# AlexanderFengler/hddm

Measured on AMD Instinct MI355X. Metric: trial-likelihood evals/sec (full DDM, sv/sz/st) at 1/2/4/8 GPUs, higher is better.
Workload: dtype f64; 1 GPU; C3: full DDM 1M trials on 1 GPU; trials_per_gpu=1000000, global_trials=1000000, parallelism=trial-shard x1

## Files before the change

hddm_amd/_lib.py:

```python
import ctypes
import os
import threading

import numpy as np

_PKG = os.path.dirname(os.path.abspath(__file__))
LIB_PATH = os.environ.get("WFPT_AMD_LIB", os.path.join(_PKG, "lib", "libwfpt_amd.so"))

if not os.path.exists(LIB_PATH):
    raise ImportError(
        f"hddm_amd: HIP library not found at {LIB_PATH}; build it with "
        "`python -m hddm_amd.build` (hipcc --offload-arch=gfx950)")

os.environ.setdefault("HIP_FORCE_DEV_KERNARG", "1")

_lib = ctypes.CDLL(LIB_PATH)

WFPT_OK = 0
WFPT_MAX_DEPTH = 24
WFPT_DS_INPUT_ORDER = 1
PATH_LEAN, PATH_ENGINE, PATH_SMALL, PATH_REDO = 1, 2, 4, 8
PATH_FOLD, PATH_DIRECT, PATH_FIXED, PATH_SPLIT = 16, 32, 64, 128
PATH_SMALL_SPLIT, PATH_NODE_SPLIT, PATH_NODE_RARE = 256, 512, 1024
LINK_IDENTITY, LINK_EXP, LINK_INVLOGIT = 0, 1, 2
# ... 71 lines not shown
    "wfpt_wiener_like_host": (_I, [_VP, _PD, _I64, _PP, _PK, _PD]),
    "wfpt_pdf_array": (_I, [_VP, _PD, _I64, _PP, _PK, _I, _PD]),
    "wfpt_full_pdf": (_I, [_VP, _D, _PP, _PK, _PD]),
    "wfpt_wiener_like_multi": (_I, [_VP, _PD, _I64] + _MULTI),
    "wfpt_wiener_like_multi_ex": (_I, [_VP, _PD, _I64] + _MULTI + [_PD]),
    "wfpt_dmat_cdf_array": (_I, [_VP, _PD, _I64, _PP, _D, _PD]),
    "wfpt_dmat_cdf_rows": (_I, [_VP, _PP, _PD, _PD, _PD, _I64, _I32, _D, _PD, _PD, _PD]),
    "wfpt_comm_unique_id": (_I, [_CP]),
    "wfpt_comm_init": (_I, [_VP, _I, _I, _CP]),
    "wfpt_comm_exchange_id": (_I, [_I, _I, _CP, _I, _I, _CP]),
    "wfpt_comm_init_tcp": (_I, [_VP, _I, _I, _CP, _I, _I]),
    "wfpt_comm_init_all": (_I, [_PVP, _I]),
    "wfpt_wiener_like_allreduce": (_I, _LIKE),
    "wfpt_wiener_like_allreduce_group": (_I, [_PVP, _PVP, _I, _PP, _PK, _PD]),
    "wfpt_wiener_like_nodes_allreduce": (_I, [_VP, _VP, _PP, _I32, _PK, _PD]),
    "wfpt_result_poison": (_I, [_PD]),
    "wfpt_decode_result": (_I, [_PD, _PD]),
    "wfpt_profile_enable": (_I, [_VP, _I]),
    "wfpt_profile_read": (_I, [_VP, _PD, _PI64, _PI64, _I]),
    "wfpt_profile_stages": (_I, [_VP, _PD, _I]),
    "wfpt_profile_lists": (_I, [_VP, _PI64, _I]),
    "wfpt_debug_waves": (_I, [_VP, _PU64, _I64]),
    "wfpt_debug_partials": (_I, [_VP, _PD, _PI32, _I64]),
    "wfpt_last_path": (_I, [_VP, _PI]),
    "wfpt_rl_dataset_create": (_I, [_VP, _PD, _PI64, _PD, _PI64, _I64, _PI32, _I32, _PVP]),
    "wfpt_rl_dataset_destroy": (None, [_VP]),
    "wfpt_wiener_like_rlddm": (_I, [_VP, _VP, _D, _D, _D, _PP, _PK, _PD]),
    "wfpt_wiener_like_rlddm_ex": (_I, [_VP, _VP, _D, _D, _D, _PP, _PK, _PD, _PD, _PD]),
    "wfpt_wiener_like_rl": (_I, [_VP, _VP] + [_D] * 7 + [_PD]),
    "wfpt_wiener_like_rl_ex": (_I, [_VP, _VP] + [_D] * 7 + [_PD, _PD, _PD]),
    "wfpt_wiener_like_multi_rlddm": (_I, _RL_HOST + _MULTI),
    "wfpt_wiener_like_multi_rlddm_ex": (_I, _RL_HOST + _MULTI + [_PD, _PD]),
    "wfpt_wiener_like_rlddm_nodes": (_I, [_VP, _VP, _PD, _PP, _PK, _PD]),
    "wfpt_wiener_like_rlddm_nodes_ex": (_I, [_VP, _VP, _PD, _PP, _PK, _PD, _PD, _PD]),
    "wfpt_wiener_like_rlddm_nodes_multi": (_I, [_VP, _VP, _PD, _PP, _I32, _PK, _PD]),
    "wfpt_wiener_like_rlddm_nodes_multi_ex": (_I, [_VP, _VP, _PD, _PP, _I32, _PK, _PD, _PD, _PD]),
    "wfpt_reg_dataset_create": (_I, [_VP, _PD, _I64, _PD, _I32, _PI32, _I32, _PVP]),
    "wfpt_reg_dataset_destroy": (None, [_VP]),
    "wfpt_wiener_like_reg": (_I, _REG),
    "wfpt_wiener_like_reg_ex": (_I, _REG + [_PD, _PD]),
    "wfpt_wiener_like_reg_groups": (_I, _REG),
    "wfpt_wiener_like_reg_groups_ex": (_I, _REG + [_PD, _PD]),
    "wfpt_rl_reg_dataset_create": (_I, [_VP, _PD, _PI64, _PD, _PI64, _I64, _PD, _I32, _PI32, _I32,
                                        _PVP]),
    "wfpt_rl_reg_dataset_destroy": (None, [_VP]),
    "wfpt_wiener_like_rl_reg_groups": (_I, _RL_REG),
# ... 130 lines not shown
        a = (_I64 * 16)()
        if wfpt_profile_lists is None:
            return {}
        check(wfpt_profile_lists(self.handle, a, 1 if reset else 0))
        v = list(a)
        return {"segments": v[0], "lean_table": v[0], "node_deferred": v[3], "lean_generic": v[3],
                "tasks1": v[1], "tasks2": v[2], "records": v[4], "exact": v[5],
                "walk": v[6], "zwalks": v[7], "zwalks0": v[8], "zwalks1": v[9],
                "zwalks2": v[10], "phase_kcycles": v[11:16]}

    def debug_waves(self, n):
        out = np.zeros((n, 8), dtype=np.uint64)
        check(wfpt_debug_waves(self.handle, out.ctypes.data_as(_PU64), n))
        return out

    def synchronize(self):
        check(wfpt_synchronize(self.handle))

    def last_path(self):
        v = _I()
        check(wfpt_last_path(self.handle, ctypes.byref(v)))
        return v.value

    def partials(self, n):
        part = np.empty(n, dtype=np.float64)
        zero = np.empty(n, dtype=np.int32)
        check(wfpt_debug_partials(self.handle, dptr(part), zero.ctypes.data_as(_PI32), n))
        return part, zero


_ctx_lock = threading.Lock()
_contexts = {}


def default_device():
    env = os.environ.get("WFPT_DEVICE")
    if env is not None:
        return int(env)
    return 0


def context(device=None):
    dev = default_device() if device is None else int(device)
    with _ctx_lock:
        c = _contexts.get(dev)
        if c is None:
# ... 26 lines not shown
```

hddm_amd/csrc/capi_core.cpp:

```cpp
#include <cstdio>

#include "capi_internal.hpp"
#include "rl_internal.h"

using namespace wfpt::capi;

constexpr int64_t kSplitCap = 16384;
constexpr int64_t kHeavyFewDiv = 16;

namespace wfpt {
namespace capi {

thread_local std::string g_last_error;

int fail(int code, const std::string& msg) {
  g_last_error = msg;
  return code;
}

bool roctx_on() {
  static const bool on = [] {
    const char* e = std::getenv("WFPT_ROCTX");
    return !(e && std::strcmp(e, "0") == 0);
  }();
  return on;
}

void ds_register(wfpt_ctx* c, DsBase* d) {
  d->ctx = c;
  c->dsets.push_back(d);
}
// ... 107 lines not shown
}

static const wfpt::DecisionTab* decision_tab_of(wfpt_ctx* c, double err) {
  uint64_t key;
  std::memcpy(&key, &err, sizeof key);
  if (!c->dtab_valid || c->dtab_err != key) {
    if (err > 1e-30 && err < 1e30) wfpt::decision_tab(err, c->dtab);
    else wfpt::decision_tab_clear(c->dtab);
    c->dtab_err = key;
    c->dtab_valid = true;
  }
  return &c->dtab;
}

int run_sum(wfpt_ctx* c, const double* dx, int64_t n, const wfpt::Params& P,
            const wfpt::Knobs& K, double* out, int part, const wfpt_ds* d,
            double* mirror) {
  const int64_t nb = wfpt::partials_for(n, P, K);
  HIP_TRY(c->part.reserve(std::max<int64_t>(nb, 1)));
  HIP_TRY(c->zero.reserve(std::max<int64_t>(nb, 1)));
  wfpt::Work W;
  if (int rc = reserve_work(c, n, &W)) return rc;
  const bool adaptive = wfpt::has_deferred_pass(P, K);
  if (part & wfpt::kPassFast) c->path = 0;
  if (c->count && (part & wfpt::kPassFast))
    HIP_TRY(hipMemsetAsync(c->evals.p, 0, sizeof(unsigned long long), c->stream));
  const bool prof = c->profile && (part & wfpt::kPassFast);
  if (prof) HIP_TRY(hipEventRecord(c->ev0, c->stream));
  const bool eng = d && d->hcount.p && engine_family(P, K) &&
                   !(part & (wfpt::kPassLean | wfpt::kPassRedo));
  const bool level0_only = adaptive && (engine_family(P, K)
                                            ? part == (wfpt::kPassFast | wfpt::kPassLean)
                                            : part == wfpt::kPassFast);
  const bool direct = adaptive && !engine_family(P, K);
  if (c->small && level0_only && !prof && !c->count && !mirror) {
    const int sk = wfpt::launch_small(dx, n, P, K, c->part.p, c->zero.p, c->status.p, W, out,
                                      c->seq + 1, c->tree_any.p, c->stream, c->trial);
    if (sk != wfpt::kSmallNone) {
      ++c->seq;
      HIP_TRY(hipGetLastError());
      c->path |= WFPT_PATH_SMALL | (direct ? WFPT_PATH_DIRECT : WFPT_PATH_LEAN) |
                 (sk == wfpt::kSmallSplit ? WFPT_PATH_SMALL_SPLIT : 0);
      return WFPT_OK;
    }
  }
  const wfpt::Split S = eng ? split_of(d) : wfpt::Split{};
  wfpt::launch_trials(c->trial ? 3 : 0, adaptive ? part : wfpt::kPassAll, dx, n, P, K, c->part.p,
                      c->zero.p, c->count ? c->evals.p : nullptr, c->status.p, 0, W, c->stream,
                      prof ? c->ev1 : nullptr, &S, c->trial,
                      ((part & wfpt::kPassLean) &&
                       wfpt::select_mode(P.sz, P.st, K.use_adaptive) == wfpt::kAdaptTZ)
                          ? decision_tab_of(c, K.err)
                          : nullptr);
  if (!adaptive) {
    c->path |= WFPT_PATH_FIXED;
  } else {
    if (part & wfpt::kPassFast)
      c->path |= direct ? WFPT_PATH_DIRECT
                        : (part & wfpt::kPassLean)
                              ? WFPT_PATH_LEAN
                              : (WFPT_PATH_ENGINE | (S.n + S.n2 > 0 ? WFPT_PATH_SPLIT : 0));
    if (!direct && (part & wfpt::kPassRedo)) c->path |= WFPT_PATH_REDO;
    if (part & wfpt::kPassDeferred) c->path |= WFPT_PATH_FOLD;
  }
  HIP_TRY(hipGetLastError());
  wfpt::launch_finalize(c->part.p, c->zero.p, nb, adaptive ? 1 : 0,
                        c->status.p, out, ++c->seq, c->stream, eng ? S.next_n : nullptr,
                        eng ? d->hcount.p + d->parity : nullptr, c->tree_any.p, mirror, c->fin.p,
                        c->fin_ticket.p);
  HIP_TRY(hipGetLastError());
  return WFPT_OK;
}

int finish_profile(wfpt_ctx* c) {
  if (c->profile) {
    float ms = 0.f;
// ... 194 lines not shown

int wfpt_open(int device, wfpt_ctx** out) {
  if (!out) return fail(WFPT_ERR_ARG, "null pointer");
  int nd = 0;
  HIP_TRY(hipGetDeviceCount(&nd));
  if (device < 0 || device >= nd)
    return fail(WFPT_ERR_ARG, "device " + std::to_string(device) + " not present (" +
                                  std::to_string(nd) + " visible)");
  DeviceGuard g(device);
  HIP_TRY(hipSetDevice(device));
  auto* c = new wfpt_ctx();
  c->device = device;
  if (const char* sm = std::getenv("WFPT_SYNC")) c->spin = std::strcmp(sm, "stream") != 0;
  if (const char* nm = std::getenv("WFPT_NODES")) c->nodes_generic = std::strcmp(nm, "generic") == 0;
  if (const char* ns = std::getenv("WFPT_NODE_SPLIT")) c->node_split = std::strcmp(ns, "0") != 0;
  if (const char* nq = std::getenv("WFPT_NODE_SPEC")) c->node_spec = std::strcmp(nq, "0") != 0;
  if (const char* ht = std::getenv("WFPT_HOST_TIMING")) c->host_timing = std::strcmp(ht, "0") != 0;
  if (const char* nt = std::getenv("WFPT_NODE_TABLE_DEV"))
    c->node_table_dev = std::strcmp(nt, "0") != 0;
  if (const char* fm = std::getenv("WFPT_FAST_ONLY")) c->fast_only = std::strcmp(fm, "0") != 0;
  if (const char* lm = std::getenv("WFPT_LEAN")) c->lean = std::strcmp(lm, "0") != 0;
  if (const char* sm = std::getenv("WFPT_SMALL")) c->small = std::strcmp(sm, "0") != 0;
  if (const char* lt = std::getenv("WFPT_LEAN_TREE")) c->lean_tree_max = std::atof(lt);
  hipError_t e = hipStreamCreateWithFlags(&c->stream, hipStreamNonBlocking);
  if (e == hipSuccess) e = hipEventCreate(&c->ev0);
  if (e == hipSuccess) e = hipEventCreate(&c->ev1);
  auto words = [&](auto& b, size_t n) {
    if (e == hipSuccess) e = b.reserve(n);
    if (e == hipSuccess) e = hipMemset(b.p, 0, n * sizeof(*b.p));
  };
  words(c->evals, 1), words(c->status, 1), words(c->n_defer, 4), words(c->ncnt, 4);
  words(c->tree_any, 1), words(c->fin, 3 * 64), words(c->fin_ticket, 1), words(c->ar, 8);
  words(c->prof, 16), words(c->phase, 8 * wfpt::kPhaseWaves);
  if (e == hipSuccess) e = c->host_status.reserve(1);
  if (e == hipSuccess) e = c->mres.reserve(8);
  if (e == hipSuccess) std::memset(c->mres.h, 0, 8 * sizeof(double));
  if (e != hipSuccess) {
    wfpt_close(c);
    return fail(WFPT_ERR_HIP, std::string("wfpt_open: ") + hipGetErrorString(e));
  }
  *out = c;
  return WFPT_OK;
}

void wfpt_close(wfpt_ctx* c) {
  if (!c) return;
// ... 57 lines not shown
    for (int64_t i = 0; i < n; ++i) ord[i] = i;
    if (!keep_order) stable_order(ord, rt, false);
    std::vector<int64_t> pos(cnt.begin(), cnt.end() - 1);
    for (int64_t q : ord) idx[pos[node_id[q]]++] = q;
  } else if (!keep_order) {
    stable_order(idx, rt, true);
  }
  std::vector<double> hx(n);
  std::vector<int32_t> hn(node_id ? n : 0);
  for (int64_t i = 0; i < n; ++i) {
    hx[i] = rt[idx[i]];
    if (node_id) hn[i] = node_id[idx[i]];
  }
  auto* d = new wfpt_ds();
  d->n = n;
  d->input_order = (flags & WFPT_DS_INPUT_ORDER) != 0;
  d->n_nodes = node_id ? n_nodes : 0;
  hipError_t e = upload_vec(d->x, hx);
  d->identity = !((!keep_order || node_id) && n > 0);
  if (e == hipSuccess && !d->identity) e = upload_vec(d->perm, idx);
  if (e == hipSuccess && node_id) e = upload_vec(d->node, hn);
  if (e == hipSuccess && node_id) e = upload_vec(d->off, off);
  d->nw = (n + 63) / 64;
  d->split_cap = (int)std::min<int64_t>(std::max<int64_t>(d->nw, 1), kSplitCap);
  const size_t cap = d->split_cap;
  auto zeroed = [&](auto& b, size_t count) {
    if (e == hipSuccess) e = b.reserve(count);
    if (e == hipSuccess) e = hipMemset(b.p, 0, count * sizeof(*b.p));
  };
  for (int k = 0; k < 2; ++k) {
    zeroed(d->hpred[k], std::max<int64_t>(d->nw, 1));
    if (e == hipSuccess) e = d->hlist[k].reserve(cap);
  }
  zeroed(d->hcount, 4);
  if (e == hipSuccess) e = d->hlp.reserve(cap * 64);
  if (e == hipSuccess) e = d->hmeta.reserve(cap * 64);
  zeroed(d->hdone, cap);
  zeroed(d->hzn, cap);
  if (e != hipSuccess) {
    delete d;
    return fail(WFPT_ERR_HIP, std::string("wfpt_dataset_create: ") + hipGetErrorString(e));
  }
  ds_register(c, d);
  *out = d;
  return WFPT_OK;
}
// ... 790 lines not shown
  HIP_TRY(hipMemcpy(ph.data(), c->phase.p, ph.size() * sizeof(ph[0]), hipMemcpyDeviceToHost));
  for (int k = 0; k < 5; ++k) {
    unsigned long long t = 0;
    for (int w = 0; w < wfpt::kPhaseWaves; ++w) t += ph[w * 8 + 2 + k];
    counts[11 + k] = (int64_t)(t / 1000);
  }
  if (reset) {
    HIP_TRY(hipMemset(c->prof.p, 0, sizeof(h)));
    HIP_TRY(hipMemset(c->phase.p, 0, ph.size() * sizeof(ph[0])));
  }
  return WFPT_OK;
}

int wfpt_debug_waves(wfpt_ctx* c, uint64_t* out, int64_t max_records) {
  if (!c || !out) return fail(WFPT_ERR_ARG, "null pointer");
  std::lock_guard<std::mutex> lk(c->mu);
  DeviceGuard g(c->device);
  HIP_TRY(hipStreamSynchronize(c->stream));
  const int64_t n = std::min<int64_t>(max_records, wfpt::kPhaseWaves);
  HIP_TRY(hipMemcpy(out, c->phase.p, n * 8 * sizeof(uint64_t), hipMemcpyDeviceToHost));
  return WFPT_OK;
}

int wfpt_synchronize(wfpt_ctx* c) {
  if (!c) return fail(WFPT_ERR_ARG, "null pointer");
  DeviceGuard g(c->device);
  HIP_TRY(hipStreamSynchronize(c->stream));
  return WFPT_OK;
}

}
```

hddm_amd/csrc/capi_internal.hpp:

```cpp
#pragma once
#include <hip/hip_runtime.h>
#include <rccl/rccl.h>
#include <rocprofiler-sdk-roctx/roctx.h>

#include <algorithm>
#include <chrono>
#include <cmath>
#include <cstdint>
#include <cstdlib>
#include <cstring>
#include <mutex>
#include <string>
#include <utility>
#include <vector>

#include "../../include/wfpt_amd.h"
#include "pointwise_internal.h"
#include "wfpt_internal.h"
#include "wfpt_lean_tables.hpp"
#include "wfpt_types.hpp"

#pragma GCC visibility push(hidden)

namespace wfpt {
// ... 212 lines not shown
  DevBuf<int> nd_chunks;
  DevBuf<int> ncnt;
  DevBuf<int> n_defer;
  DevBuf<unsigned long long> evals;
  DevBuf<int> status;
  MappedBuf<int> host_status;
  MappedBuf<double> mres;
  unsigned long long seq = 0;
  MappedBuf<wfpt::Params> mnodep;
  DevBuf<wfpt::Params> dnodep;
  bool host_timing = false;
  std::chrono::steady_clock::time_point ht_mark;
  double ht[5] = {0, 0, 0, 0, 0};
  int64_t ht_calls = 0;
  bool node_table_dev = false;
  MappedBuf<double> mnode;
  bool spin = true;
  bool nodes_generic = false;
  bool node_split = false;
  bool node_spec = true;
  bool fast_only = true;
  bool lean = true;
  bool small = true;
  double lean_tree_max = 0.0;
  bool profile = false;
  bool count = false;
  double k_ms = 0.0;
  int64_t launches = 0;
  int64_t n_evals = 0;
  double* trial = nullptr;
  int path = 0;
  hipEvent_t ev0 = nullptr, ev1 = nullptr;
  ncclComm_t comm = nullptr;
  int nranks = 1, rank = 0;
  std::vector<wfpt::capi::DsBase*> dsets;
  wfpt::capi::RlWork rl;
  wfpt::capi::RegWork reg;
  wfpt::capi::SimWork sim;
  wfpt::capi::StatsWork stats;
  wfpt::capi::PointwiseWork pw;
};

struct wfpt_ds : wfpt::capi::DsBase {
  int64_t n = 0;
  DevBuf<double> x;
  DevBuf<int32_t> node;
  DevBuf<int64_t> off;
  int32_t n_nodes = 0;
  mutable bool no_defer = false;
  mutable bool no_tree = false;
  mutable double tree_frac = 1.0;
  bool input_order = false;
  int64_t nw = 0;
  int split_cap = 0;
  DevBuf<unsigned char> hpred[2];
  DevBuf<int> hlist[2];
  DevBuf<int> hcount;
  DevBuf<double> hlp;
  DevBuf<int> hmeta;
  DevBuf<int> hdone;
  DevBuf<int> hzn;
  mutable int nsplit = 0;
  mutable int nsplit2 = 0;
  mutable int parity = 0;
  DevBuf<int64_t> perm;
  bool identity = true;
  void free_device() override {
    wfpt::capi::release_all(x, node, off, perm, hpred[0], hpred[1], hlist[0], hlist[1], hcount,
                            hlp, hmeta, hdone, hzn);
  }
};

namespace wfpt {
namespace capi {

inline Params to_params(const wfpt_params* p) {
  return Params{p->v, p->sv, p->a, p->z, p->sz, p->t, p->st, p->p_outlier};
}
inline Knobs to_knobs(const wfpt_knobs* k) {
  return Knobs{k->err, k->n_st, k->n_sz, k->use_adaptive != 0, k->simps_err, k->w_outlier};
}
inline bool p_outlier_in_range(double p) { return (p >= 0) & (p <= 1); }

int begin_status(wfpt_ctx* c);
int fetch_status(wfpt_ctx* c);
int check_status(wfpt_ctx* c);
int check_status_value(double enc);
bool engine_family(const Params& P, const Knobs& K);
// ... 50 lines not shown
```

hddm_amd/csrc/wfpt_internal.h:

```cpp
#pragma once
#include <hip/hip_runtime.h>
#include <stdint.h>

#include <algorithm>
#include <type_traits>

#include "../../include/wfpt_amd.h"
#include "wfpt_lean_tables.hpp"
#include "wfpt_types.hpp"

namespace wfpt {

struct Work {
  unsigned char* wl;
  int* wl_n;
  int* rflag;
  int* prof;
  unsigned long long* phase;
  unsigned char* redo;
  int* tree_any;
  int64_t nslots;
};

constexpr int kPhaseWaves = 16384;
// ... 10 lines not shown
  const unsigned char* pred;
  unsigned char* next_pred;
  int* next_list;
  int* next_n;
  double* lp;
  int* meta;
  int* done;
  int* zn;
};

constexpr double kBudgetUnit = 1048576.0;
constexpr double kPeerFailUnit = 1099511627776.0;

int stack_kind(const Knobs& K);
int64_t blocks_for(int64_t n);
bool has_deferred_pass(const Params& P, const Knobs& K);
int64_t partials_for(int64_t n, const Params& P, const Knobs& K);

constexpr int kPassFast = 1, kPassDeferred = 2, kPassAll = 3, kPassLean = 4, kPassRedo = 8;
void launch_trials(int out_kind, int part, const double* x, int64_t n, const Params& P,
                   const Knobs& K, double* out, int* zeros, unsigned long long* evals, int* status,
                   int logp, const Work& W, hipStream_t s, hipEvent_t fast_done = nullptr,
                   const Split* split = nullptr, double* trial = nullptr,
                   const DecisionTab* dtab = nullptr);
constexpr int kResDeferred = 1, kResTree = 2;
void launch_finalize(const double* part, const int* zeros, int64_t nb, int defer_bits,
                     int* status, double* out, unsigned long long seq, hipStream_t s,
                     const int* split_rd = nullptr, int* split_rs = nullptr,
                     int* tree_any = nullptr, double* mirror = nullptr,
                     double* fin = nullptr, int* ticket = nullptr);
constexpr int kSmallNone = 0, kSmallOne = 1, kSmallSplit = 2;
int launch_small(const double* x, int64_t n, const Params& P, const Knobs& K, double* part,
                 int* zeros, int* status, const Work& W, double* out, unsigned long long seq,
                 int* tree_any, hipStream_t s, double* trial = nullptr);
void launch_publish(const double* res, double* out, unsigned long long seq, hipStream_t s);
void launch_poison(double* res, hipStream_t s);
struct NodeTables {
  int32_t n_nodes;
  bool split, spec;
  int32_t n_tables = 1;
  int64_t* rare_v = nullptr;
  int32_t* rare_j = nullptr;
};
struct NodeSum {
  const double* x;
  const int32_t* node;
  const Params* P;
// ... 41 lines not shown
```

hddm_amd/csrc/wfpt_kernel_common.hpp:

```cpp
#pragma once
#include <cstdio>
#include <cstdlib>

#include "wfpt_grid.hpp"
#include "wfpt_internal.h"
#include "wfpt_lean_tables.hpp"
#include "wfpt_level0.hpp"
#include "wfpt_math.hpp"
#include "wfpt_quad.hpp"
#include "wfpt_series.hpp"
#include "wfpt_types.hpp"
#include "wfpt_zgrid.hpp"

#pragma clang fp contract(off)

namespace wfpt {

constexpr int kBlock = 256;
constexpr int kFastBlock = 256;
static inline int64_t fast_blocks(int64_t n) { return (n + kFastBlock - 1) / kFastBlock; }

#ifndef WFPT_FAST_WAVES
#define WFPT_FAST_WAVES 3
#endif
// ... 216 lines not shown
}
template <bool ARRAY, class F>
inline void with_build(bool count, int out, F&& f) {
  if (out == OUT_SUM) {
    with_flag(count, [&](auto c) { f(c, std::integral_constant<int, OUT_SUM>{}); });
    return;
  }
  if (count) bad_dispatch("a counting build of out kind", out);
  if (out == OUT_BOTH) {
    f(std::false_type{}, std::integral_constant<int, OUT_BOTH>{});
    return;
  }
  if constexpr (ARRAY) {
    if (out == OUT_ARRAY) {
      f(std::false_type{}, std::integral_constant<int, OUT_ARRAY>{});
      return;
    }
  }
  bad_dispatch("out kind", out);
}

void launch_direct(bool count, int out, const TrialArgs& A, const Work& W, hipStream_t s);
void launch_lean(int mode, bool count, int out, const TrialArgs& A, const Work& W, hipStream_t s,
                 const DecisionTab* dt);
void launch_engine(int mode, bool count, int out, const TrialArgs& A, const Work& W,
                   const EngTables& T, const Split& S, hipStream_t s);
void launch_fold(int mode, bool count, int out, const TrialArgs& A, const Work& W, hipStream_t s);

}
```

hddm_amd/csrc/wfpt_lean.hpp:

```cpp
#pragma once
#include <hip/hip_runtime.h>

#include "wfpt_grid.hpp"
#include "wfpt_lean_tables.hpp"
#include "wfpt_level0.hpp"
#include "wfpt_math.hpp"
#include "wfpt_quad.hpp"
#include "wfpt_series.hpp"
#include "wfpt_types.hpp"
#include "wfpt_zgrid.hpp"

#pragma clang fp contract(off)

namespace wfpt {

__device__ inline bool table_decisions(const DecisionTab& D, double xs, double lb, double ub,
                                       double ia2, unsigned long long own, int lane,
                                       unsigned& kpack, unsigned& smask) {
  kpack = 0u;
  smask = 0u;
  const double prev = __shfl_up(xs, 1);
  const bool mine = ((own >> lane) & 1ull) != 0ull;
  if (__ballot(mine && !(prev <= xs)) != 0ull) return false;
  const int last = __popcll(own) - 1;
  const double xmin = __hiloint2double(__builtin_amdgcn_readlane(__double2hiint(xs), 0),
                                       __builtin_amdgcn_readlane(__double2loint(xs), 0));
  const double xmax = __hiloint2double(__builtin_amdgcn_readlane(__double2hiint(xs), last),
                                       __builtin_amdgcn_readlane(__double2loint(xs), last));
  const double e = D.edge[lane];
  const double c = (ub + lb) / 2.;
  const double d = (lb + c) / 2., f = (c + ub) / 2.;
  bool ok = true;
#pragma unroll
  for (int j = 0; j < 5; ++j) {
    const double tc = j == 0 ? lb : j == 1 ? d : j == 2 ? c : j == 3 ? f : ub;
    const int n0 = __popcll(__ballot(e <= (xmin - tc) * ia2));
    const int n1 = __popcll(__ballot(e <= (xmax - tc) * ia2));
    const unsigned code = D.code[(n0 >> 1) & (kDecPieces - 1)];
    ok = ok && n0 == n1 && (n0 & 1) != 0 && code != 0u;
    kpack |= (code & 15u) << (4 * j);
    smask |= ((code >> 4) & 1u) << j;
  }
  return ok;
}

__device__ inline bool l0_decisions(const Trial& tr, const Params& P, const Knobs& K, L0Hints& H,
                                    unsigned& kpack, unsigned& smask) {
  kpack = 0u;
  smask = 0u;
  double lb, ub;
  tree_root<kAdaptTZ>(tr, P, lb, ub);
  H = l0_hints(tr.x, lb, ub, P.a, K.err);
  bool ok = tr.valid && (tr.x - ub > 0) && H.q0 >= 0.0 && H.ok0 && H.ok4;
  if (!ok) return false;
  const double c = (ub + lb) / 2.;
  const double d = (lb + c) / 2., e = (c + ub) / 2.;
  auto put = [&](int j, const Decision& D) {
    ok = ok && D.amb == 0 && D.K >= 1 && D.K <= (D.small ? kUniK : kSinK);
    kpack |= (unsigned)(D.K & 15) << (4 * j);
    smask |= (D.small ? 1u : 0u) << j;
  };
  put(0, H.D0);
  put(4, H.D4);
  if (H.shared) {
    put(1, H.D0);
    put(2, H.D0);
// ... 160 lines not shown
```

hddm_amd/csrc/wfpt_lean_tables.hpp:

```cpp
#pragma once
#include <hip/hip_runtime.h>

#include "wfpt_types.hpp"
#include "wfpt_zgrid.hpp"

#pragma clang fp contract(off)

namespace wfpt {

constexpr int kUniK = 8;
static_assert(kSinK <= 15 && kUniK <= 15, "K packs into 4 bits per t node");
struct UniformK {
  double u0u0;
  double hh2;
  double hh;
  double u0p1;
  double h;
  double bound;
};
struct UniformTab {
  double u[9][5];
  UniformK k[kUniK + 1];
  double amax;
};
// ... 105 lines not shown
      for (;;) {
        const double m = l + (r - l) * 0.5;
        if (!(l < m && m < r)) break;
        if (decision_code(m, err) == ca) l = m;
        else r = m;
      }
      emit(start, l * (1.0 - kDecBand), ca);
      start = r * (1.0 + kDecBand);
      a = r;
      ca = decision_code(r, err);
    }
    a = b;
  }
  emit(start, hi, ca);
  if (full) decision_tab_clear(T);
}
inline unsigned decision_lookup(const DecisionTab& T, double tt, int* count = nullptr) {
  int n = 0;
  for (int e = 0; e < 2 * kDecPieces; ++e) n += T.edge[e] <= tt ? 1 : 0;
  if (count) *count = n;
  return (n & 1) ? T.code[(n >> 1) & (kDecPieces - 1)] : 0u;
}

}
```

hddm_amd/csrc/wfpt_level0.hip:

```cpp
#include "wfpt_kernel_common.hpp"
#include "wfpt_lean.hpp"

#pragma clang fp contract(off)

namespace wfpt {

template <bool COUNT, int OUT>
__global__ __launch_bounds__(kFastBlock, FastWaves<kDirect>::value > 0 ? FastWaves<kDirect>::value : 1)
void direct_kernel(TrialArgs A, Work W, DirectArgs D) {
  const int64_t i = (int64_t)blockIdx.x * kFastBlock + threadIdx.x;
  const int lane = threadIdx.x & 63;
  const int64_t c = i >> 6;
  if (c * 64 >= A.n) return;
  const bool own = i < A.n;
  const double x0 = own ? A.x[i] : 0.0;
  double p = 0.0;
  long long ne = 0;
  int flags = 0, oc = kFinal;
  const bool pos = x0 > 0;
  const unsigned long long bo = __ballot(own), bp = __ballot(own && pos);
  const int b = (bp == bo) ? 1 : 0;
  if (own && pos == (b != 0)) oc = direct_level0(x0, A.P, A.K, D, b, p, ne, flags);
  if (bp != 0ull && bp != bo) {
    if (own && pos) oc = direct_level0(x0, A.P, A.K, D, 1, p, ne, flags);
// ... 2 lines not shown
  int zero = 0;
  if (own && oc == kFinal) emit<OUT>(A, i, p, lp, zero);
  const bool anyd = defer_slots(W, c, lane, oc != kFinal, kFlagExact);
  if (sum_out(OUT)) {
    lp = wave_sum(lp);
    const int zs = __popcll(__ballot(zero != 0));
    if (lane == 0) {
      A.out[c] = lp;
      A.zeros[c] = zs | (anyd ? kZeroDefer : 0);
    }
  }
  if (COUNT) {
    const long long nf = wave_sum_ll(oc == kFinal ? ne : 0);
    if (lane == 0) atomicAdd(A.evals, (unsigned long long)nf);
  }
}

#ifndef WFPT_LEAN_BLOCK
#define WFPT_LEAN_BLOCK 256
#endif
constexpr int kLeanBlock = WFPT_LEAN_BLOCK;
static_assert(kLeanBlock % 64 == 0 && kLeanBlock <= kFastBlock, "kLeanBlock");
static_assert(sizeof(TrialArgs) + sizeof(Work) + sizeof(RootGrids) + sizeof(UniformTabs) +
                      sizeof(DecisionTab) <= 4096,
              "lean_kernel's arguments exceed the 4 KB kernel argument segment");
template <int MODE, bool COUNT, int OUT>
__global__ __launch_bounds__(kLeanBlock, FastWaves<MODE>::value > 0 ? FastWaves<MODE>::value : 1)
void lean_kernel(TrialArgs A, Work W, RootGrids R, UniformTabs T, DecisionTab D) {
#ifdef WFPT_PHASE_TIMING
  const long long rt0 = __builtin_amdgcn_s_memrealtime();
#endif
  const int64_t i = (int64_t)blockIdx.x * kLeanBlock + threadIdx.x;
  const int lane = threadIdx.x & 63;
  const int64_t c = i >> 6;
  if (c * 64 >= A.n) return;
  const bool own = i < A.n;
  const double x0 = own ? A.x[i] : 0.0;
  double p = 0.0, f0[5] = {0.0, 0.0, 0.0, 0.0, 0.0};
  long long ne0 = 0;
  unsigned pend0 = 0u;
  int oc = kFinal;
  const bool pos = x0 > 0;
  const unsigned long long bo = __ballot(own), bp = __ballot(own && pos);
  const int b = (bp == bo) ? 1 : 0;
  bool done = false;
  if constexpr (MODE == kAdaptTZ) {
    if (bp == bo || bp == 0ull) {
      const Trial tr = trial_setup_b(x0, A.P, b != 0);
      double lb, ub;
      tree_root<MODE>(tr, A.P, lb, ub);
      L0Hints H;
      unsigned kp0, sm0;
      H.q0 = -1.0;
      H.R = 0.0;
      H.ia2 = 1.0 / (A.P.a * A.P.a);
      H.D0 = H.D4 = Decision{0, 0, 0};
      H.ok0 = H.ok4 = H.shared = false;
      bool tab = __ballot(own && tr.valid && tr.x - ub > 0) == bo &&
                 table_decisions(D, tr.x, lb, ub, H.ia2, bo, lane, kp0, sm0);
      if (tab && sm0 != 31u) {
        const double q0 = exp_node((-kPi2 * ((tr.x - lb) * H.ia2)) * 0.5);
        const double Rr = exp_node((kPi2 * (ub - lb)) * (0.125 * H.ia2));
        H.q0 = q0;
        H.R = Rr;
        tab = __ballot(own && q0 > 1e-280 && Rr < 1e10) == bo;
      }
      bool uni = tab;
      if (!tab) {
        unsigned kp, sm;
        const bool okd = own && l0_decisions(tr, A.P, A.K, H, kp, sm);
        kp0 = __builtin_amdgcn_readfirstlane(kp);
        sm0 = __builtin_amdgcn_readfirstlane(sm);
        uni = __ballot(okd && kp == kp0 && sm == sm0) == bo;
      }
      if (uni) {
        int kmax = 0;
#pragma unroll
        for (int j = 0; j < 5; ++j) {
          const int kj = (int)((kp0 >> (4 * j)) & 15u);
          if (((sm0 >> j) & 1u) != 0u && kj > kmax) kmax = kj;
        }
        const UniformTab& U = T.U[b];
        const bool safe = uniform_guard((tr.x - ub) * H.ia2, (tr.v * tr.v) * (tr.x - lb), A.P.sv,
                                        U.k[kmax].bound, U.amax);
        if (__ballot(own && safe) == bo) {
          bool bail = false;
          if (own)
            oc = lean_uniform_level0(tr, A.P, A.K, zgrid_uniform(R, b), U, &R.S[b][0][0], H, kp0,
                                     sm0, p, ne0, pend0, bail);
          done = __ballot(own && bail) == 0ull;
          if (COUNT && done && tab && lane == 0) atomicAdd(&W.prof[0], 1);
        }
      }
    }
  }
  if (!done) {
    p = 0.0;
    ne0 = 0;
    pend0 = 0u;
    oc = kFinal;
    if (own && pos == (b != 0))
      oc = eng_level0_t<MODE, false, true>(trial_setup_b(x0, A.P, b != 0), A.P, A.K,
                                           zgrid_uniform(R, b), p, f0, ne0, pend0, &R.S[b][0][0]);
    if (bp != 0ull && bp != bo) {
      if (own && pos)
        oc = eng_level0_t<MODE, false, true>(trial_setup_b(x0, A.P, true), A.P, A.K, R.G[1], p, f0,
                                             ne0, pend0, &R.S[1][0][0]);
    }
    if (COUNT && MODE == kAdaptTZ && lane == 0) atomicAdd(&W.prof[3], 1);
  }
  if (__ballot(oc == kTree) != 0ull) {
    if (lane == 0) {
      W.redo[c] = 1;
      if (sum_out(OUT)) A.zeros[c] = kZeroDefer;
    }
    return;
  }
  chunk_out<COUNT, OUT>(A, W, c, lane, p, oc == kExact, kFlagExact, ne0);
#ifdef WFPT_PHASE_TIMING
  if (lane == 0 && c < kPhaseWaves) {
    unsigned long long* rec = W.phase + c * 8;
    rec[0] = rt0;
    rec[1] = __builtin_amdgcn_s_memrealtime();
    unsigned hw;
    asm volatile("s_getreg_b32 %0, hwreg(HW_REG_HW_ID)" : "=s"(hw));
    rec[2] = hw;
    unsigned xcc;
    asm volatile("s_getreg_b32 %0, hwreg(HW_REG_XCC_ID)" : "=s"(xcc));
    rec[3] = xcc;
  }
#endif
}


void launch_direct(bool count, int out, const TrialArgs& A, const Work& W, hipStream_t s) {
  DirectArgs D;
  direct_args(A.P, D);
  with_build<true>(count, out, [&](auto c, auto o) {
    hipLaunchKernelGGL((direct_kernel<decltype(c)::value, decltype(o)::value>),
                       dim3(fast_blocks(A.n)), dim3(kFastBlock), 0, s, A, W, D);
  });
}

void launch_lean(int mode, bool count, int out, const TrialArgs& A, const Work& W, hipStream_t s,
                 const DecisionTab* dt) {
  DecisionTab D;
  if (dt) D = *dt;
  else decision_tab_clear(D);
  RootGrids R;
  root_grids(A.P, R);
  UniformTabs T;
  uniform_tabs(R, T);
  with_value<kAdaptT, kAdaptTZ>(mode, [&](auto m) {
    with_build<false>(count, out, [&](auto c, auto o) {
      hipLaunchKernelGGL((lean_kernel<decltype(m)::value, decltype(c)::value, decltype(o)::value>),
                         dim3((A.n + kLeanBlock - 1) / kLeanBlock), dim3(kLeanBlock), 0, s, A, W, R,
                         T, D);
    });
  });
}

}
```

hddm_amd/csrc/wfpt_sum.hip:

```cpp
#include "wfpt_kernel_common.hpp"

#pragma clang fp contract(off)

namespace wfpt {

constexpr int kFinLoads = 16;
constexpr int kFinMaxBlocks = 64;
constexpr int64_t kFinPerBlock = 8192;
__global__ __launch_bounds__(1024) void finalize_kernel(const double* part, const int* zeros,
                                                        int64_t nb, int defer_bits,
                                                        int* status, double* out,
                                                        unsigned long long seq,
                                                        const int* split_rd, int* split_rs,
                                                        int* tree_any, double* mirror,
                                                        double* fin, int* ticket) {
  __shared__ double ss[16];
  __shared__ long long sz[16];
  __shared__ int sd[16];
  __shared__ int last;
  const int G = gridDim.x;
  int64_t lo = 0, hi = nb;
  if (G > 1) {
    const int64_t L = (nb + G - 1) / G;
    lo = (int64_t)blockIdx.x * L;
// ... 386 lines not shown

int64_t blocks_for(int64_t n) { return (n + kBlock - 1) / kBlock; }

bool has_deferred_pass(const Params& P, const Knobs& K) {
  return select_mode(P.sz, P.st, K.use_adaptive) <= kAdaptTZ;
}

int64_t partials_for(int64_t n, const Params& P, const Knobs& K) {
  return has_deferred_pass(P, K) ? (n + 63) / 64 : blocks_for(n);
}

static void launch_fixed(int mode, bool count, int out, const TrialArgs& A, hipStream_t s) {
  with_value<kFixedT, kFixedTZ>(mode, [&](auto m) {
    with_build<true>(count, out, [&](auto c, auto o) {
      hipLaunchKernelGGL((trial_kernel<decltype(m)::value, decltype(c)::value, decltype(o)::value>),
                         dim3(blocks_for(A.n)), dim3(kBlock), 0, s, A);
    });
  });
}

void launch_trials(int out_kind, int part, const double* x, int64_t n, const Params& P,
                   const Knobs& K, double* out, int* zeros, unsigned long long* evals, int* status,
                   int logp, const Work& W, hipStream_t s, hipEvent_t fast_done,
                   const Split* split, double* trial, const DecisionTab* dtab) {
  if (n <= 0) return;
  Split S{};
  if (split) S = *split;
  const TrialArgs A = trial_args(x, n, P, K, out, zeros, evals, status, logp, trial);
  const int mode = select_mode(P.sz, P.st, K.use_adaptive);
  const bool count = evals && out_kind == OUT_SUM;
  if (mode > kAdaptTZ) {
    launch_fixed(mode, count, out_kind, A, s);
    if (fast_done) (void)hipEventRecord(fast_done, s);
    return;
  }
  EngTables T;
  const bool engine = ((part & kPassFast) && !(part & kPassLean)) || (part & kPassRedo);
  if (mode != kDirect && engine) eng_tables(A.P, T);
  Work F = W;
  F.redo = (part & (kPassLean | kPassRedo)) ? W.redo : nullptr;
  if (part & kPassFast) {
    if (mode == kDirect) launch_direct(count, out_kind, A, F, s);
    else if (part & kPassLean) launch_lean(mode, count, out_kind, A, F, s, dtab);
    else launch_engine(mode, count, out_kind, A, F, T, S, s);
    if (fast_done) (void)hipEventRecord(fast_done, s);
  }
  if (part & kPassDeferred) {
    if (mode != kDirect && (part & kPassRedo)) launch_engine(mode, count, out_kind, A, F, T, Split{}, s);
    launch_fold(mode, count, out_kind, A, F, s);
  }
}

int launch_small(const double* x, int64_t n, const Params& P, const Knobs& K, double* part,
                 int* zeros, int* status, const Work& W, double* out, unsigned long long seq,
                 int* tree_any, hipStream_t s, double* trial) {
  if (n <= 0 || n > kFastBlock) return kSmallNone;
  const int mode = select_mode(P.sz, P.st, K.use_adaptive);
  if (mode > kAdaptTZ) return kSmallNone;
  const TrialArgs A = trial_args(x, n, P, K, part, zeros, nullptr, status, 0, trial);
  Work F = W;
  F.redo = mode == kDirect ? nullptr : W.redo;
  RootGrids R{};
  if (mode != kDirect) root_grids(P, R);
  const FinArgs Fa{status, out, seq, tree_any, 1};
  with_build<false>(false, trial ? OUT_BOTH : OUT_SUM, [&](auto, auto o) {
    constexpr int O = decltype(o)::value;
// ... 37 lines not shown
```

include/wfpt_amd.h:

```cpp
#ifndef WFPT_AMD_H
#define WFPT_AMD_H

#include <stdint.h>

#ifdef __cplusplus
extern "C" {
#endif

#define WFPT_OK 0
#define WFPT_ERR_HIP 1
#define WFPT_ERR_ARG 2
#define WFPT_ERR_COMM 3
#define WFPT_ERR_UNSUPPORTED 4

#define WFPT_MAX_DEPTH 24
#define WFPT_EVAL_BUDGET (1ll << 24)

typedef struct wfpt_ctx wfpt_ctx;
typedef struct wfpt_ds wfpt_ds;

typedef struct wfpt_params {
    double v, sv, a, z, sz, t, st, p_outlier;
} wfpt_params;

// ... 256 lines not shown
                             const double *u_choice, const double *u_delay, uint64_t seed,
                             int64_t workspace_bytes, double *out, const double *q, int32_t nq,
                             double *stats_out);
int wfpt_gen_rts_drift_nodes_stats(wfpt_ctx *ctx, const wfpt_params *rows, int64_t R,
                                   const double *sw, const int64_t *counts, double dt,
                                   double intra_sv, int64_t max_steps, uint64_t seed,
                                   double *out, int64_t *n_unfinished, const double *q,
                                   int32_t nq, double *stats_out);

int wfpt_gen_rlddm_rows_stats(wfpt_ctx *ctx, const wfpt_params *rows, const double *rl_rows,
                              int64_t R, const int64_t *counts, const wfpt_rl_source *source,
                              double dt, double intra_sv, int64_t max_steps, uint64_t seed,
                              double *out, int64_t *n_unfinished, const int64_t *group_off,
                              int64_t n_groups, const double *q, int32_t nq, double *stats_out);

int wfpt_profile_stages(wfpt_ctx *ctx, double stage_ms[4], int reset);
#define WFPT_PROF_EVENTS 1
#define WFPT_PROF_EVALS 2
int wfpt_profile_enable(wfpt_ctx *ctx, int flags);
int wfpt_profile_read(wfpt_ctx *ctx, double *kernel_ms, int64_t *launches, int64_t *n_evals,
                      int reset);
int wfpt_profile_lists(wfpt_ctx *ctx, int64_t counts[16], int reset);
int wfpt_debug_waves(wfpt_ctx *ctx, uint64_t *out, int64_t max_records);
int wfpt_debug_partials(wfpt_ctx *ctx, double *part, int32_t *zero, int64_t n);
#define WFPT_PATH_LEAN 1
#define WFPT_PATH_ENGINE 2
#define WFPT_PATH_SMALL 4
#define WFPT_PATH_REDO 8
#define WFPT_PATH_FOLD 16
#define WFPT_PATH_DIRECT 32
#define WFPT_PATH_FIXED 64
#define WFPT_PATH_SPLIT 128
#define WFPT_PATH_SMALL_SPLIT 256
#define WFPT_PATH_NODE_SPLIT 512
#define WFPT_PATH_NODE_RARE 1024
int wfpt_last_path(wfpt_ctx *ctx, int *path);
int wfpt_synchronize(wfpt_ctx *ctx);

#ifdef __cplusplus
}
#endif
#endif
```

Baseline: 14.84 billion trials/s.

## Schedule slow lean-kernel chunks first and add a split-decision table shortcut

A host-side sorted index of chunk-first RTs is built at dataset creation. Per call, a binary search predicts which 64-trial chunks straddle decision-table boundaries, and those chunks are remapped to run first in the lean kernel. This is meant to shrink the tail from slow waves that would otherwise land last. A table_split check also lets waves whose decisions differ across the chunk skip the per-lane l0_decisions path. The remapping is active only when the wave count falls between the device's slot count and eight times that. It adds host search work on every call and a larger kernel argument block.

```diff
diff --git a/hddm_amd/_lib.py b/hddm_amd/_lib.py
--- a/hddm_amd/_lib.py
+++ b/hddm_amd/_lib.py
@@ -117,6 +117,7 @@
     "wfpt_profile_lists": (_I, [_VP, _PI64, _I]),
     "wfpt_debug_waves": (_I, [_VP, _PU64, _I64]),
     "wfpt_debug_partials": (_I, [_VP, _PD, _PI32, _I64]),
+    "wfpt_debug_lean_first": (_I, [_VP, _PI32, _I32, _PI32]),
     "wfpt_last_path": (_I, [_VP, _PI]),
     "wfpt_rl_dataset_create": (_I, [_VP, _PD, _PI64, _PD, _PI64, _I64, _PI32, _I32, _PVP]),
     "wfpt_rl_dataset_destroy": (None, [_VP]),
@@ -293,6 +294,12 @@
         check(wfpt_last_path(self.handle, ctypes.byref(v)))
         return v.value
 
+    def lean_first(self):
+        out = np.zeros(64, dtype=np.int32)
+        n = _I32()
+        check(wfpt_debug_lean_first(self.handle, out.ctypes.data_as(_PI32), 64, ctypes.byref(n)))
+        return [int(v) for v in out[:n.value]]
+
     def partials(self, n):
         part = np.empty(n, dtype=np.float64)
         zero = np.empty(n, dtype=np.int32)
diff --git a/hddm_amd/csrc/capi_core.cpp b/hddm_amd/csrc/capi_core.cpp
--- a/hddm_amd/csrc/capi_core.cpp
+++ b/hddm_amd/csrc/capi_core.cpp
@@ -7,6 +7,7 @@
 
 constexpr int64_t kSplitCap = 16384;
 constexpr int64_t kHeavyFewDiv = 16;
+constexpr int64_t kLeanFirstRounds = 8;
 
 namespace wfpt {
 namespace capi {
@@ -160,7 +161,10 @@
   wfpt::Work W;
   if (int rc = reserve_work(c, n, &W)) return rc;
   const bool adaptive = wfpt::has_deferred_pass(P, K);
-  if (part & wfpt::kPassFast) c->path = 0;
+  if (part & wfpt::kPassFast) {
+    c->path = 0;
+    c->first_last.n = 0;
+  }
   if (c->count && (part & wfpt::kPassFast))
     HIP_TRY(hipMemsetAsync(c->evals.p, 0, sizeof(unsigned long long), c->stream));
   const bool prof = c->profile && (part & wfpt::kPassFast);
@@ -183,13 +187,17 @@
     }
   }
   const wfpt::Split S = eng ? split_of(d) : wfpt::Split{};
+  const bool lean2d = (part & wfpt::kPassLean) &&
+                      wfpt::select_mode(P.sz, P.st, K.use_adaptive) == wfpt::kAdaptTZ;
+  if (lean2d && c->lean_first && d && d->lean_index.first && d->nw > c->lean_first_min &&
+      d->nw <= c->lean_first_max)
+    wfpt::lean_first_search(*decision_tab_of(c, K.err), d->lean_index, P.a, P.t, P.st,
+                            c->first_last);
   wfpt::launch_trials(c->trial ? 3 : 0, adaptive ? part : wfpt::kPassAll, dx, n, P, K, c->part.p,
                       c->zero.p, c->count ? c->evals.p : nullptr, c->status.p, 0, W, c->stream,
                       prof ? c->ev1 : nullptr, &S, c->trial,
-                      ((part & wfpt::kPassLean) &&
-                       wfpt::select_mode(P.sz, P.st, K.use_adaptive) == wfpt::kAdaptTZ)
-                          ? decision_tab_of(c, K.err)
-                          : nullptr);
+                      lean2d ? decision_tab_of(c, K.err) : nullptr,
+                      lean2d ? &c->first_last : nullptr);
   if (!adaptive) {
     c->path |= WFPT_PATH_FIXED;
   } else {
@@ -430,6 +438,13 @@
   if (const char* lm = std::getenv("WFPT_LEAN")) c->lean = std::strcmp(lm, "0") != 0;
   if (const char* sm = std::getenv("WFPT_SMALL")) c->small = std::strcmp(sm, "0") != 0;
   if (const char* lt = std::getenv("WFPT_LEAN_TREE")) c->lean_tree_max = std::atof(lt);
+  if (const char* lf = std::getenv("WFPT_LEAN_FIRST")) c->lean_first = std::strcmp(lf, "0") != 0;
+  {
+    const int64_t slots = wfpt::lean_wave_slots();
+    c->lean_first_min = slots > 0 ? slots : INT64_MAX;
+    c->lean_first_max = slots > 0 ? slots * kLeanFirstRounds : 0;
+    if (const char* fm = std::getenv("WFPT_LEAN_FIRST_MIN")) c->lean_first_min = std::atoll(fm);
+  }
   hipError_t e = hipStreamCreateWithFlags(&c->stream, hipStreamNonBlocking);
   if (e == hipSuccess) e = hipEventCreate(&c->ev0);
   if (e == hipSuccess) e = hipEventCreate(&c->ev1);
@@ -533,6 +548,10 @@
   if (e == hipSuccess && node_id) e = upload_vec(d->node, hn);
   if (e == hipSuccess && node_id) e = upload_vec(d->off, off);
   d->nw = (n + 63) / 64;
+  if (!node_id && !keep_order && n > 0) {
+    d->chunk_first.resize(d->nw);
+    wfpt::lean_index(hx.data(), n, d->chunk_first.data(), d->lean_index);
+  }
   d->split_cap = (int)std::min<int64_t>(std::max<int64_t>(d->nw, 1), kSplitCap);
   const size_t cap = d->split_cap;
   auto zeroed = [&](auto& b, size_t count) {
@@ -1369,6 +1388,15 @@
   return WFPT_OK;
 }
 
+int wfpt_debug_lean_first(wfpt_ctx* c, int32_t* chunks, int32_t max_chunks, int32_t* n) {
+  if (!c || !n || (max_chunks > 0 && !chunks) || max_chunks < 0)
+    return fail(WFPT_ERR_ARG, "bad arguments");
+  std::lock_guard<std::mutex> lk(c->mu);
+  *n = c->first_last.n;
+  for (int k = 0; k < c->first_last.n && k < max_chunks; ++k) chunks[k] = c->first_last.c[k];
+  return WFPT_OK;
+}
+
 int wfpt_synchronize(wfpt_ctx* c) {
   if (!c) return fail(WFPT_ERR_ARG, "null pointer");
   DeviceGuard g(c->device);
diff --git a/hddm_amd/csrc/capi_internal.hpp b/hddm_amd/csrc/capi_internal.hpp
--- a/hddm_amd/csrc/capi_internal.hpp
+++ b/hddm_amd/csrc/capi_internal.hpp
@@ -258,6 +258,9 @@
   bool fast_only = true;
   bool lean = true;
   bool small = true;
+  bool lean_first = true;
+  int64_t lean_first_min = 0, lean_first_max = 0;
+  wfpt::LeanFirst first_last{};
   double lean_tree_max = 0.0;
   bool profile = false;
   bool count = false;
@@ -300,6 +303,8 @@
   mutable int nsplit2 = 0;
   mutable int parity = 0;
   DevBuf<int64_t> perm;
+  std::vector<double> chunk_first;
+  wfpt::LeanIndex lean_index{};
   bool identity = true;
   void free_device() override {
     wfpt::capi::release_all(x, node, off, perm, hpred[0], hpred[1], hlist[0], hlist[1], hcount,
diff --git a/hddm_amd/csrc/wfpt_internal.h b/hddm_amd/csrc/wfpt_internal.h
--- a/hddm_amd/csrc/wfpt_internal.h
+++ b/hddm_amd/csrc/wfpt_internal.h
@@ -56,7 +56,8 @@
                    const Knobs& K, double* out, int* zeros, unsigned long long* evals, int* status,
                    int logp, const Work& W, hipStream_t s, hipEvent_t fast_done = nullptr,
                    const Split* split = nullptr, double* trial = nullptr,
-                   const DecisionTab* dtab = nullptr);
+                   const DecisionTab* dtab = nullptr, const LeanFirst* first = nullptr);
+int64_t lean_wave_slots();
 constexpr int kResDeferred = 1, kResTree = 2;
 void launch_finalize(const double* part, const int* zeros, int64_t nb, int defer_bits,
                      int* status, double* out, unsigned long long seq, hipStream_t s,
diff --git a/hddm_amd/csrc/wfpt_kernel_common.hpp b/hddm_amd/csrc/wfpt_kernel_common.hpp
--- a/hddm_amd/csrc/wfpt_kernel_common.hpp
+++ b/hddm_amd/csrc/wfpt_kernel_common.hpp
@@ -262,7 +262,7 @@
 
 void launch_direct(bool count, int out, const TrialArgs& A, const Work& W, hipStream_t s);
 void launch_lean(int mode, bool count, int out, const TrialArgs& A, const Work& W, hipStream_t s,
-                 const DecisionTab* dt);
+                 const DecisionTab* dt, const LeanFirst* first = nullptr);
 void launch_engine(int mode, bool count, int out, const TrialArgs& A, const Work& W,
                    const EngTables& T, const Split& S, hipStream_t s);
 void launch_fold(int mode, bool count, int out, const TrialArgs& A, const Work& W, hipStream_t s);
diff --git a/hddm_amd/csrc/wfpt_lean.hpp b/hddm_amd/csrc/wfpt_lean.hpp
--- a/hddm_amd/csrc/wfpt_lean.hpp
+++ b/hddm_amd/csrc/wfpt_lean.hpp
@@ -42,6 +42,33 @@
     smask |= ((code >> 4) & 1u) << j;
   }
   return ok;
+}
+
+__device__ inline bool table_split(const DecisionTab& D, double xs, double lb, double ub,
+                                   double ia2, unsigned long long own, int lane) {
+  const double prev = __shfl_up(xs, 1);
+  const bool mine = ((own >> lane) & 1ull) != 0ull;
+  if (__ballot(mine && !(prev <= xs)) != 0ull) return false;
+  const int last = __popcll(own) - 1;
+  const double xmin = __hiloint2double(__builtin_amdgcn_readlane(__double2hiint(xs), 0),
+                                       __builtin_amdgcn_readlane(__double2loint(xs), 0));
+  const double xmax = __hiloint2double(__builtin_amdgcn_readlane(__double2hiint(xs), last),
+                                       __builtin_amdgcn_readlane(__double2loint(xs), last));
+  const double e = D.edge[lane];
+  const double c = (ub + lb) / 2.;
+  const double d = (lb + c) / 2., f = (c + ub) / 2.;
+  bool inside = true, differ = false;
+#pragma unroll 1
+  for (int j = 0; j < 5; ++j) {
+    const double tc = j == 0 ? lb : j == 1 ? d : j == 2 ? c : j == 3 ? f : ub;
+    const int n0 = __popcll(__ballot(e <= (xmin - tc) * ia2));
+    const int n1 = __popcll(__ballot(e <= (xmax - tc) * ia2));
+    const unsigned c0 = D.code[(n0 >> 1) & (kDecPieces - 1)];
+    const unsigned c1 = D.code[(n1 >> 1) & (kDecPieces - 1)];
+    inside = inside && (n0 & 1) != 0 && (n1 & 1) != 0 && c0 != 0u && c1 != 0u;
+    differ = differ || (n0 != n1 && c0 != c1);
+  }
+  return inside && differ;
 }
 
 __device__ inline bool l0_decisions(const Trial& tr, const Params& P, const Knobs& K, L0Hints& H,
diff --git a/hddm_amd/csrc/wfpt_lean_tables.hpp b/hddm_amd/csrc/wfpt_lean_tables.hpp
--- a/hddm_amd/csrc/wfpt_lean_tables.hpp
+++ b/hddm_amd/csrc/wfpt_lean_tables.hpp
@@ -151,4 +151,87 @@
   return (n & 1) ? T.code[(n >> 1) & (kDecPieces - 1)] : 0u;
 }
 
-}
+constexpr int kLeanFirstMax = 64;
+struct LeanFirst {
+  int n;
+  int c[kLeanFirstMax];
+};
+struct LeanIndex {
+  const double* first;
+  int64_t nw;
+  int64_t lower_n;
+  int64_t upper;
+  int64_t n;
+  double upper_first;
+  double last[2];
+};
+inline void lean_index(const double* x, int64_t n, double* first, LeanIndex& I) {
+  const int64_t nw = (n + 63) / 64;
+  for (int64_t w = 0; w < nw; ++w) first[w] = __builtin_fabs(x[w * 64]);
+  int64_t up = 0;
+  while (up < n && !(x[up] > 0)) ++up;
+  int64_t ln = up;
+  while (ln > 0 && x[ln - 1] != x[ln - 1]) --ln;
+  I.first = first;
+  I.nw = nw;
+  I.n = n;
+  I.upper = up;
+  I.lower_n = ln;
+  I.upper_first = up < n ? __builtin_fabs(x[up]) : 0.0;
+  I.last[0] = ln > 0 ? __builtin_fabs(x[ln - 1]) : 0.0;
+  I.last[1] = up < n ? __builtin_fabs(x[n - 1]) : 0.0;
+}
+inline int64_t lean_chunk_of(const LeanIndex& I, int b, double r) {
+  int64_t lo, hi;
+  double k0;
+  if (b == 0) {
+    if (I.lower_n <= 0) return -1;
+    lo = 0;
+    hi = (I.lower_n + 63) / 64;
+    k0 = I.first[0];
+  } else {
+    if (I.upper >= I.n) return -1;
+    lo = I.upper / 64;
+    hi = I.nw;
+    k0 = I.upper_first;
+  }
+  if (!(r >= k0 && r <= I.last[b])) return -1;
+  int64_t l = lo, h = hi;
+  while (h - l > 1) {
+    const int64_t m = l + (h - l) / 2;
+    if (I.first[m] <= r) l = m;
+    else h = m;
+  }
+  return l;
+}
+inline void lean_first_search(const DecisionTab& D, const LeanIndex& I, double a, double t,
+                              double st, LeanFirst& F) {
+  F.n = 0;
+  for (int k = 0; k < kLeanFirstMax; ++k) F.c[k] = 0;
+  if (!I.first || I.nw <= 0) return;
+  const double lb = t - st / 2., ub = t + st / 2.;
+  const double c = (ub + lb) / 2.;
+  const double tc[5] = {lb, (lb + c) / 2., c, (c + ub) / 2., ub};
+  const double a2 = a * a;
+  int64_t cand[2 * 5 * kDecPieces];
+  int nc = 0;
+  for (int b = 0; b < 2; ++b)
+    for (int j = 0; j < 5; ++j)
+      for (int p = 0; p < kDecPieces; ++p) {
+        const double e = D.edge[2 * p + 1];
+        if (!(e < __builtin_inf())) continue;
+        const int64_t ch = lean_chunk_of(I, b, tc[j] + e * a2);
+        if (ch < 0) continue;
+        int q = nc;
+        while (q > 0 && cand[q - 1] > ch) --q;
+        if (q > 0 && cand[q - 1] == ch) continue;
+        for (int s = nc; s > q; --s) cand[s] = cand[s - 1];
+        cand[q] = ch;
+        ++nc;
+      }
+  const int skip = nc > kLeanFirstMax ? nc - kLeanFirstMax : 0;
+  F.n = nc - skip;
+  for (int k = 0; k < F.n; ++k) F.c[k] = (int)cand[skip + k];
+}
+
+}
diff --git a/hddm_amd/csrc/wfpt_level0.hip b/hddm_amd/csrc/wfpt_level0.hip
--- a/hddm_amd/csrc/wfpt_level0.hip
+++ b/hddm_amd/csrc/wfpt_level0.hip
@@ -48,18 +48,32 @@
 constexpr int kLeanBlock = WFPT_LEAN_BLOCK;
 static_assert(kLeanBlock % 64 == 0 && kLeanBlock <= kFastBlock, "kLeanBlock");
 static_assert(sizeof(TrialArgs) + sizeof(Work) + sizeof(RootGrids) + sizeof(UniformTabs) +
-                      sizeof(DecisionTab) <= 4096,
+                      sizeof(DecisionTab) + sizeof(LeanFirst) <= 4096,
               "lean_kernel's arguments exceed the 4 KB kernel argument segment");
-template <int MODE, bool COUNT, int OUT>
+template <int MODE, bool COUNT, int OUT, bool FIRST>
 __global__ __launch_bounds__(kLeanBlock, FastWaves<MODE>::value > 0 ? FastWaves<MODE>::value : 1)
-void lean_kernel(TrialArgs A, Work W, RootGrids R, UniformTabs T, DecisionTab D) {
+void lean_kernel(TrialArgs A, Work W, RootGrids R, UniformTabs T, DecisionTab D, LeanFirst F) {
 #ifdef WFPT_PHASE_TIMING
   const long long rt0 = __builtin_amdgcn_s_memrealtime();
 #endif
-  const int64_t i = (int64_t)blockIdx.x * kLeanBlock + threadIdx.x;
   const int lane = threadIdx.x & 63;
+  int64_t i = (int64_t)blockIdx.x * kLeanBlock + threadIdx.x;
+  if constexpr (FIRST) {
+    const int w = (int)(i >> 6);
+    if (w < F.n) {
+      i = (int64_t)F.c[w] * 64 + lane;
+    } else {
+      const int listed = F.c[lane];
+      if (__ballot(lane < F.n && listed == w - F.n) != 0ull) return;
+      i -= (int64_t)F.n * 64;
+    }
+  }
   const int64_t c = i >> 6;
   if (c * 64 >= A.n) return;
+#ifdef WFPT_PHASE_TIMING
+  if (FIRST && lane == 0 && c < kPhaseWaves)
+    W.phase[c * 8 + 5] = ((unsigned long long)blockIdx.x * kLeanBlock + threadIdx.x) >> 6;
+#endif
   const bool own = i < A.n;
   const double x0 = own ? A.x[i] : 0.0;
   double p = 0.0, f0[5] = {0.0, 0.0, 0.0, 0.0, 0.0};
@@ -70,6 +84,9 @@
   const unsigned long long bo = __ballot(own), bp = __ballot(own && pos);
   const int b = (bp == bo) ? 1 : 0;
   bool done = false;
+#ifdef WFPT_PHASE_TIMING
+  int site = 2;
+#endif
   if constexpr (MODE == kAdaptTZ) {
     if (bp == bo || bp == 0ull) {
       const Trial tr = trial_setup_b(x0, A.P, b != 0);
@@ -82,8 +99,8 @@
       H.ia2 = 1.0 / (A.P.a * A.P.a);
       H.D0 = H.D4 = Decision{0, 0, 0};
       H.ok0 = H.ok4 = H.shared = false;
-      bool tab = __ballot(own && tr.valid && tr.x - ub > 0) == bo &&
-                 table_decisions(D, tr.x, lb, ub, H.ia2, bo, lane, kp0, sm0);
+      const bool pre = __ballot(own && tr.valid && tr.x - ub > 0) == bo;
+      bool tab = pre && table_decisions(D, tr.x, lb, ub, H.ia2, bo, lane, kp0, sm0);
       if (tab && sm0 != 31u) {
         const double q0 = exp_node((-kPi2 * ((tr.x - lb) * H.ia2)) * 0.5);
         const double Rr = exp_node((kPi2 * (ub - lb)) * (0.125 * H.ia2));
@@ -92,7 +109,7 @@
         tab = __ballot(own && q0 > 1e-280 && Rr < 1e10) == bo;
       }
       bool uni = tab;
-      if (!tab) {
+      if (!tab && !(pre && table_split(D, tr.x, lb, ub, H.ia2, bo, lane))) {
         unsigned kp, sm;
         const bool okd = own && l0_decisions(tr, A.P, A.K, H, kp, sm);
         kp0 = __builtin_amdgcn_readfirstlane(kp);
@@ -115,6 +132,9 @@
             oc = lean_uniform_level0(tr, A.P, A.K, zgrid_uniform(R, b), U, &R.S[b][0][0], H, kp0,
                                      sm0, p, ne0, pend0, bail);
           done = __ballot(own && bail) == 0ull;
+#ifdef WFPT_PHASE_TIMING
+          if (done) site = tab ? 0 : 1;
+#endif
           if (COUNT && done && tab && lane == 0) atomicAdd(&W.prof[0], 1);
         }
       }
@@ -154,6 +174,7 @@
     unsigned xcc;
     asm volatile("s_getreg_b32 %0, hwreg(HW_REG_XCC_ID)" : "=s"(xcc));
     rec[3] = xcc;
+    rec[4] = (unsigned long long)site;
   }
 #endif
 }
@@ -169,7 +190,7 @@
 }
 
 void launch_lean(int mode, bool count, int out, const TrialArgs& A, const Work& W, hipStream_t s,
-                 const DecisionTab* dt) {
+                 const DecisionTab* dt, const LeanFirst* first) {
   DecisionTab D;
   if (dt) D = *dt;
   else decision_tab_clear(D);
@@ -177,13 +198,39 @@
   root_grids(A.P, R);
   UniformTabs T;
   uniform_tabs(R, T);
+  LeanFirst F;
+  F.n = 0;
+  for (int k = 0; k < kLeanFirstMax; ++k) F.c[k] = 0;
+  const int64_t nw = (A.n + 63) / 64;
+  if (first && mode == kAdaptTZ && first->n > 0 && first->n <= kLeanFirstMax) {
+    bool ok = true;
+    for (int k = 0; k < first->n; ++k)
+      ok = ok && first->c[k] >= 0 && first->c[k] < nw && (k == 0 || first->c[k] > first->c[k - 1]);
+    if (ok) F = *first;
+  }
+  const int64_t waves = nw + F.n, per = kLeanBlock / 64;
+  const dim3 grid((waves + per - 1) / per);
   with_value<kAdaptT, kAdaptTZ>(mode, [&](auto m) {
     with_build<false>(count, out, [&](auto c, auto o) {
-      hipLaunchKernelGGL((lean_kernel<decltype(m)::value, decltype(c)::value, decltype(o)::value>),
-                         dim3((A.n + kLeanBlock - 1) / kLeanBlock), dim3(kLeanBlock), 0, s, A, W, R,
-                         T, D);
+      if (F.n > 0)
+        hipLaunchKernelGGL((lean_kernel<kAdaptTZ, decltype(c)::value, decltype(o)::value, true>),
+                           grid, dim3(kLeanBlock), 0, s, A, W, R, T, D, F);
+      else
+        hipLaunchKernelGGL(
+            (lean_kernel<decltype(m)::value, decltype(c)::value, decltype(o)::value, false>), grid,
+            dim3(kLeanBlock), 0, s, A, W, R, T, D, F);
     });
   });
 }
 
-}
+int64_t lean_wave_slots() {
+  int dev = 0, cus = 0, blocks = 0;
+  if (hipGetDevice(&dev) != hipSuccess ||
+      hipDeviceGetAttribute(&cus, hipDeviceAttributeMultiprocessorCount, dev) != hipSuccess ||
+      hipOccupancyMaxActiveBlocksPerMultiprocessor(
+          &blocks, lean_kernel<kAdaptTZ, false, OUT_SUM, true>, kLeanBlock, 0) != hipSuccess)
+    return 0;
+  return (int64_t)cus * blocks * (kLeanBlock / 64);
+}
+
+}
diff --git a/hddm_amd/csrc/wfpt_sum.hip b/hddm_amd/csrc/wfpt_sum.hip
--- a/hddm_amd/csrc/wfpt_sum.hip
+++ b/hddm_amd/csrc/wfpt_sum.hip
@@ -432,7 +432,8 @@
 void launch_trials(int out_kind, int part, const double* x, int64_t n, const Params& P,
                    const Knobs& K, double* out, int* zeros, unsigned long long* evals, int* status,
                    int logp, const Work& W, hipStream_t s, hipEvent_t fast_done,
-                   const Split* split, double* trial, const DecisionTab* dtab) {
+                   const Split* split, double* trial, const DecisionTab* dtab,
+                   const LeanFirst* first) {
   if (n <= 0) return;
   Split S{};
   if (split) S = *split;
@@ -451,7 +452,7 @@
   F.redo = (part & (kPassLean | kPassRedo)) ? W.redo : nullptr;
   if (part & kPassFast) {
     if (mode == kDirect) launch_direct(count, out_kind, A, F, s);
-    else if (part & kPassLean) launch_lean(mode, count, out_kind, A, F, s, dtab);
+    else if (part & kPassLean) launch_lean(mode, count, out_kind, A, F, s, dtab, first);
     else launch_engine(mode, count, out_kind, A, F, T, S, s);
     if (fast_done) (void)hipEventRecord(fast_done, s);
   }
diff --git a/include/wfpt_amd.h b/include/wfpt_amd.h
--- a/include/wfpt_amd.h
+++ b/include/wfpt_amd.h
@@ -302,6 +302,7 @@
                       int reset);
 int wfpt_profile_lists(wfpt_ctx *ctx, int64_t counts[16], int reset);
 int wfpt_debug_waves(wfpt_ctx *ctx, uint64_t *out, int64_t max_records);
+int wfpt_debug_lean_first(wfpt_ctx *ctx, int32_t *chunks, int32_t max_chunks, int32_t *n);
 int wfpt_debug_partials(wfpt_ctx *ctx, double *part, int32_t *zero, int64_t n);
 #define WFPT_PATH_LEAN 1
 #define WFPT_PATH_ENGINE 2
```

Measured after the change: 15.62 billion trials/s, median of 6. +5.3%, better.
